# zsc/ARTalk

Hardware: AMD Instinct MI355X
Metric: motion frames/sec (25 fps clips) at batch=32 per GPU (higher is better)
Workload: dtype f32 (operands split into 2 fp16, 3 fp16 MFMA products per fp32 product, fp32 accumulate)

## Files before the change

artalk_amd/capi.py:

```python
from __future__ import annotations

import ctypes as C
import os

from .config import ARTalkConfig

_HERE = os.path.dirname(os.path.abspath(__file__))
LIB_PATH = os.environ.get("ARTALK_LIB") or os.path.join(_HERE, "libartalk_hip.so")

OK, EINVAL, EKEY, EMISSING, EHIP, ESTATE, ECAPACITY, EBUSY = 0, -1, -2, -3, -4, -5, -6, -7
DTYPE_F32, DTYPE_I64 = 0, 1

SYMBOLS = [
    "artalk_create", "artalk_destroy", "artalk_last_error", "artalk_set_tensor", "artalk_finalize_weights",
    "artalk_reserve", "artalk_workspace_bytes", "artalk_weight_bytes", "artalk_infer", "artalk_get_status", "artalk_poll_status", "artalk_last_ticket", "artalk_get_status_of", "artalk_style_encode", "artalk_stream_begin", "artalk_stream_chunk", "artalk_stream_end", "artalk_savgol", "artalk_flame_create", "artalk_flame_verts", "artalk_flame_destroy", "artalk_flame_last_error",
    "artalk_set_profiling", "artalk_get_profile", "artalk_get_kernel_sums", "artalk_set_graphs", "artalk_graph_count", "artalk_set_cu_mask", "artalk_set_audit", "artalk_get_audit", "artalk_calibrate", "artalk_reset_scales", "artalk_get_scales", "artalk_scale_sites", "artalk_get_site_scales", "artalk_set_site_scales", "artalk_set_tap", "artalk_tap_layout", "artalk_set_precision",
    "artalk_op_gemm", "artalk_op_gemm_ex", "artalk_op_gemm_bf16", "artalk_op_gemm_f16s", "artalk_op_pack_split", "artalk_op_gemm_f16s_packed", "artalk_op_release_scratch", "artalk_op_gemm_p8_plan", "artalk_op_create_masked_stream", "artalk_op_destroy_stream", "artalk_op_mfma_f32_peak", "artalk_op_layernorm", "artalk_op_attention", "artalk_op_w2v_front", "artalk_op_resample_mean", "artalk_op_pool_silu",
    "artalk_op_bsq_history",
    "artalk_sessions_reserve", "artalk_session_open", "artalk_session_step", "artalk_session_close", "artalk_session_count",
    "artalk_session_smooth", "artalk_op_savgol_stream", "artalk_op_session_smooth_check",
    "artalk_op_pack_split_ex", "artalk_op_layernorm_ex", "artalk_op_gemm_f16s_packed_ex", "artalk_op_gemm_f16s_ex", "artalk_op_attention_ex", "artalk_op_w2v_front_ex", "artalk_op_pool_silu_ex", "artalk_op_posconv_p8_ex",
    "artalk_op_bsq_history_ex", "artalk_op_ar_bits_next", "artalk_op_vq_embed", "artalk_op_ar_begin", "artalk_op_dec_input", "artalk_op_dec_finish", "artalk_op_enc_input_zero", "artalk_op_style_input", "artalk_op_add_row", "artalk_op_style_finish", "artalk_op_broadcast16", "artalk_op_session_gather", "artalk_op_session_scatter", "artalk_op_absmax",
    "artalk_op_gemm_rows", "artalk_op_layernorm_rows", "artalk_op_attention_rows", "artalk_op_gemm_rows_layout", "artalk_op_rows_dry_run",
    "artalk_op_w2v_front_rows", "artalk_op_pool_silu_rows", "artalk_op_posconv_rows",
]


class ArtalkConfigStruct(C.Structure):
    _fields_ = [
        ("ar_depth", C.c_int32), ("ar_heads", C.c_int32),
        ("vae_depth", C.c_int32), ("vae_heads", C.c_int32), ("vae_hidden", C.c_int32),
        ("code_dim", C.c_int32), ("motion_dim", C.c_int32),
        ("n_levels", C.c_int32), ("patch_nums", C.c_int32 * 8),
        ("w2v_layers", C.c_int32), ("w2v_hidden", C.c_int32), ("w2v_heads", C.c_int32), ("w2v_ffn", C.c_int32),
        ("w2v_n_conv", C.c_int32), ("w2v_conv_kernel", C.c_int32 * 8), ("w2v_conv_stride", C.c_int32 * 8),
        ("w2v_conv_dim", C.c_int32),
        ("w2v_pos_kernel", C.c_int32), ("w2v_pos_groups", C.c_int32),
        ("w2v_ln_eps", C.c_float),
        ("style_dim", C.c_int32), ("style_heads", C.c_int32), ("style_layers", C.c_int32), ("style_ffn", C.c_int32),
# ... 79 lines not shown
    L.artalk_destroy.restype = None
    L.artalk_last_error.argtypes = [vp]
    L.artalk_last_error.restype = C.c_char_p
    L.artalk_set_tensor.argtypes = [vp, C.c_char_p, vp, i32, i32, C.POINTER(i64)]
    L.artalk_set_tensor.restype = i32
    L.artalk_finalize_weights.argtypes = [vp]
    L.artalk_finalize_weights.restype = i32
    L.artalk_reserve.argtypes = [vp, i32, i32]
    L.artalk_reserve.restype = i32
    L.artalk_workspace_bytes.argtypes = [vp]
    L.artalk_workspace_bytes.restype = i64
    L.artalk_weight_bytes.argtypes = [vp]
    L.artalk_weight_bytes.restype = i64
    L.artalk_infer.argtypes = [vp, vp, i64, C.POINTER(i64), i32, vp, vp, vp, i64, vp, vp, vp, vp]
    L.artalk_infer.restype = i32
    L.artalk_get_status.argtypes = [vp, C.POINTER(C.c_int), vp]
    L.artalk_get_status.restype = i32
    L.artalk_poll_status.argtypes = [vp, C.POINTER(C.c_int)]
    L.artalk_poll_status.restype = i32
    L.artalk_last_ticket.argtypes = [vp]
    L.artalk_last_ticket.restype = C.c_longlong
    L.artalk_get_status_of.argtypes = [vp, C.c_longlong, C.POINTER(C.c_int)]
    L.artalk_get_status_of.restype = i32
    L.artalk_style_encode.argtypes = [vp, vp, i32, vp, vp]
    L.artalk_style_encode.restype = i32
    L.artalk_stream_begin.argtypes = [vp, i32, vp, vp, vp]
    L.artalk_stream_begin.restype = i32
    L.artalk_stream_end.argtypes = [vp]
    L.artalk_stream_end.restype = i32
    L.artalk_stream_chunk.argtypes = [vp, vp, i64, vp, i64, vp]
# ... 173 lines not shown
```

artalk_amd/csrc/engine.hip:

```cpp
#include "kernels.h"
#include "../../include/artalk_hip.h"

#include <hip/hip_ext.h>
#include <rocprofiler-sdk-roctx/roctx.h>

#include <algorithm>
#include <cmath>
#include <cstdio>
#include <cstdlib>
#include <cstring>
#include <map>
#include <set>
#include <string>
#include <vector>

using namespace artalk;

namespace artalk {
thread_local KernelTimer* g_ktimer = nullptr;
bool ktimer_events(hipEvent_t* e0, hipEvent_t* e1) {
    KernelTimer* t = g_ktimer;
    if (!t) return false;
    while (t->pool.size() < t->used + 2) {
        hipEvent_t e = nullptr;
// ... 116 lines not shown
        std::vector<float*> blocks;
        std::vector<int64_t> owner;
        struct Open { int slot = 0; int64_t seen = 0; bool smooth_done = false; };
        std::map<int64_t, Open> open;
        std::set<int64_t> ended_by_scales;
        int64_t next_id = 1;
        void* smooth_tab = nullptr; int64_t smooth_cap = 0;
    } sess;
    int64_t sess_carry_off() const { return slot_carry_off(cfg.code_dim); }
    int64_t sess_slot_floats() const { return sess_carry_off() + (kSavgolCarry * (int64_t)cfg.motion_dim + 3) / 4 * 4; }
    float* sess_slot(int i) const { return sess.blocks[i / kSessBlock] + (int64_t)(i % kSessBlock) * sess_slot_floats(); }
    Workspace* view = nullptr;
    bool sticky_error = false;
    int n_conv = 0; int conv_T[8]{}; int conv_S[8]{};
    int Tw = 0, Ts = 0;
    int ada_n = 0;
    int pn[kMaxLv]{}, off[kMaxLv + 1]{};
    float *conv0_w = nullptr, *conv_b[8]{}, *conv_lnw[8]{}, *conv_lnb[8]{}, *conv_w[8]{};
    float *fp_lnw = nullptr, *fp_lnb = nullptr, *fp_w = nullptr, *fp_b = nullptr;
    float *pos_w = nullptr, *pos_b = nullptr, *enc_lnw = nullptr, *enc_lnb = nullptr;
    std::vector<W2VLayer> w2v;
    float *ada_w = nullptr, *ada_b = nullptr;
    float *ar_qkv_w = nullptr, *ar_qkv_b = nullptr;
    std::vector<ARLayer> ar;
    float *logits_w = nullptr, *logits_b = nullptr, *vq_w = nullptr, *vq_b = nullptr, *sc_w = nullptr, *sc_b = nullptr;
    float *null_style = nullptr, *lvl_pos = nullptr, *prev_lvl_pos = nullptr;
    float *enc_pos = nullptr, *dec_pos = nullptr, *vae_mean = nullptr, *vae_std = nullptr;
    VAESide enc, dec;
    float *st_mean = nullptr, *st_std = nullptr, *st_pe = nullptr, *st_proj_w = nullptr, *st_proj_b = nullptr;
    std::vector<StyleLayer> style;
// ... 274 lines not shown
    auto st = m->site_of.find(ex);
    if (st == m->site_of.end()) { m->err = "internal: audited exponent is not in the site table"; m->sticky_error = true; return; }
    const std::string& name = m->sites[st->second].name;
    auto it = m->audit_index.find(name);
    int idx;
    if (it == m->audit_index.end()) {
        if ((int)m->audit_names.size() >= kAuditSlots) return;
        idx = (int)m->audit_names.size();
        m->audit_names.push_back(name);
        m->audit_exp.push_back(ex);
        m->audit_index.emplace(name, idx);
    } else idx = it->second;
    launch_absmax(buf, rows, cols & ~7, ld, is_p8 ? 1 : 0, m->audit_vals + idx, s, junk_period, junk_from, ex ? *ex : kActExp);
}

bool gemm(artalk_model* m, const GemmArgs& g0, hipStream_t s, const LnArgs* fuse_ln = nullptr) {
    GemmArgs g = g0;
    g.graph_tag = m->in_body ? 1 : 0;
    g.cus = m->n_cus;
    g.status = m->precision == 1 ? (m->view ? m->view->status : m->ws.status) : nullptr;
    if (m->precision == 1 && !g.exact) g.Wp = packed_of(m, g.W);
    if (m->precision == 2 && !g.exact) {
        g.Wb = bf16_of(m, g.W);
        if (!g.Wb || ((unsigned long long)g.Wb & 15) || (g.ldw & 7)) {
            m->err = "internal: bf16 GEMM without an aligned bf16 weight copy"; m->sticky_error = true; return false;
        }
        if (g.a_packed) { m->err = "internal: P8 activation handed to a bf16 GEMM"; m->sticky_error = true; return false; }
    }
    const Workspace& cw = m->view ? *m->view : m->ws;
    const GemmPolicy pol{m->precision, false, cw.splitk, cw.splitk_floats, m->splitk_tiles, m->splitk_target};
    const GemmPlan plan = plan_gemm(g, pol, fuse_ln);
    if (g.a_packed && plan.path == GEMM_F32) { m->err = "internal: P8 activation handed to an fp32 GEMM"; m->sticky_error = true; return false; }
    const bool timed = m->profiling && plan.dominant && !m->in_body;
    size_t i0 = 0, i1 = 0;
    if (timed) next_event(m, s, &i0);
    run_gemm(g, plan, fuse_ln, s);
    if (timed) {
        next_event(m, s, &i1);
        m->dom_events.emplace_back(i0, gemm_flops(g));
    }
    return plan.fused_ln;
}

enum { TAP_BLK0_IN = 0, TAP_BLK0_OUT = kNTok * kE, TAP_BLKL_OUT = 2 * kNTok * kE, TAP_PREV_IN = 3 * kNTok * kE,
       TAP_LOGITS = 4 * kNTok * kE, TAP_DEC_OUT = 4 * kNTok * kE + kNTok * 64, TAP_SLOT = 4 * kNTok * kE + kNTok * 64 + 200 * 106 };
void tap_copy(artalk_model* m, int field, int row0, const float* src, int rows, int cols, int B, hipStream_t s) {
    if (!m->tap || m->in_graph_body || m->tap_chunk >= m->tap_maxch || B > m->tap_B) return;
    float* dst = m->tap + ((long)m->tap_chunk * m->tap_B) * TAP_SLOT + field + (long)row0 * cols;
    (void)hipMemcpy2DAsync(dst, (size_t)TAP_SLOT * 4, src, (size_t)rows * cols * 4, (size_t)rows * cols * 4, B, hipMemcpyDeviceToDevice, s);
}

enum { LF_EXACT = 1, LF_A_P8 = 2, LF_C_P8 = 4 };
void linear(artalk_model* m, const float* A, long lda, const float* W, const float* bias, float* C, long ldc, int M, int N, int K,
            int act, const float* R, hipStream_t s, int flags = 0, float* c2 = nullptr, int a_exp = kActExp, int c_exp = kActExp) {
    GemmArgs g;
    g.c2 = c2; g.a_exp = a_exp; g.c_exp = c_exp;
    g.exact = flags & LF_EXACT; g.a_packed = (flags & LF_A_P8) ? 1 : 0; g.c_p8 = (flags & LF_C_P8) ? 1 : 0;
    g.A = A; g.lda = lda; g.W = W; g.ldw = K; g.bias = bias; g.C = C; g.ldc = ldc; g.M = M; g.N = N; g.K = K; g.act = act;
    g.R = R; g.ldr = ldc;
    gemm(m, g, s);
}

void layernorm(const float* X, float* Y, const float* w, const float* b, int M, int D, float eps, int act, hipStream_t s, int out_p8 = 0,
               int* status = nullptr, int junk_period = 0, int junk_from = 0, int p8_exp = kActExp) {
    LnArgs a;
    a.out_p8 = out_p8; a.p8_exp = p8_exp; a.status = out_p8 ? status : nullptr; a.junk_period = junk_period; a.junk_from = junk_from;
    a.X = X; a.ldx = D; a.Y = Y; a.ldy = D; a.w = w; a.b = b; a.M = M; a.D = D; a.eps = eps; a.act = act;
    launch_layernorm(a, s);
}

void run_wav2vec(artalk_model* m, const float* audio, int c0, int n, float* out_w2v, hipStream_t s) {
    const artalk_config& c = m->cfg;
    Workspace& w = m->ws;
    const int CD = c.w2v_conv_dim, Hs = c.w2v_hidden;
    const int p8 = m->precision == 1 ? 1 : 0;
    const int AP = p8 ? LF_A_P8 : 0;
    Range r_w2v("artalk.wav2vec2");
    roctxRangePushA("artalk.wav2vec2.conv_stack");
    kbucket(m, KB_CONV);
    launch_audio_normalize(audio, w.src_off + c0, w.xnorm, n, kSamplesPerChunk, s);
    SiteExps& ex = m->ex;
    launch_conv0(w.xnorm, kSamplesPerChunk, m->conv0_w, m->conv_b[0], m->conv_lnw[0], m->conv_lnb[0], w.convA, n, m->conv_T[0],
                 m->conv_S[0], s, p8, w.status, ex.conv[0]);
    audit(m, w.convA, n * m->conv_S[0], CD, CD, p8, s, &ex.conv[0], m->conv_S[0], m->conv_T[0]);
    float* src = w.convA; float* dst = w.convB;
    for (int i = 1; i < c.w2v_n_conv; ++i) {
        const int M = n * m->conv_S[i];
        linear(m, src, (long)c.w2v_conv_stride[i] * CD, m->conv_w[i], m->conv_b[i], dst, CD, M, CD, c.w2v_conv_kernel[i] * CD,
               ACT_NONE, nullptr, s, AP, nullptr, ex.conv[i - 1]);
        layernorm(dst, dst, m->conv_lnw[i], m->conv_lnb[i], M, CD, 1e-5f, ACT_GELU_ERF, s, (p8 && i + 1 < c.w2v_n_conv) ? 1 : 0, w.status,
                  m->conv_S[i], m->conv_T[i], ex.conv[i]);
        if (i + 1 < c.w2v_n_conv) audit(m, dst, M, CD, CD, p8, s, &ex.conv[i], m->conv_S[i], m->conv_T[i]);
        std::swap(src, dst);
    }
    stage_mark(m, s, PB_CONV);
    roctxRangePop();
    Range r_enc("artalk.wav2vec2.encoder");
    kbucket(m, KB_ENC);
    const int M = n * m->Ts;
    const int JP = m->Ts, JF = m->Tw;
    layernorm(src, dst, m->fp_lnw, m->fp_lnb, M, CD, c.w2v_ln_eps, ACT_NONE, s, p8, w.status, JP, JF, ex.fp_ln);
    audit(m, dst, M, CD, CD, p8, s, &ex.fp_ln, JP, JF);
    linear(m, dst, CD, m->fp_w, m->fp_b, w.h0, Hs, M, Hs, CD, ACT_NONE, nullptr, s, AP, nullptr, ex.fp_ln);
    audit(m, w.h0, M, Hs, Hs, false, s, &ex.posconv_in, JP, JF);
    {
        const int cg = Hs / c.w2v_pos_groups;
        GemmArgs g;
        g.A = w.h0; g.lda = Hs; g.W = m->pos_w; g.ldw = (long)cg * c.w2v_pos_kernel; g.bias = m->pos_b; g.C = w.h1; g.ldc = Hs; g.R = w.h0; g.ldr = Hs;
        g.M = M; g.act = ACT_GELU_ERF; g.a_exp = ex.posconv_in;
// ... 537 lines not shown
        if (m->stream_B > 0) { m->stream_B = 0; m->stream_scales_ended = true; }
        end_sessions_by_scales(m);
        m->ex = next;
    }
    m->scales_changed = 0;
    for (size_t i = 0; i < sizeof(SiteExps) / sizeof(int); ++i) m->scales_changed += a[i] != kActExp;
    return changed;
}

int call_stream(artalk_model* m, void* stream, hipStream_t* s) {
    (void)hipSetDevice(m->device);
    if (!stream && !m->own_stream) HIPCHK(m, hipStreamCreate(&m->own_stream));
    *s = stream ? (hipStream_t)stream : m->own_stream;
    return ARTALK_OK;
}
int check_has_style(artalk_model* m, const float* style_motion_dev, const uint8_t* has_style, int B, bool* encode) {
    *encode = false;
    for (int b = 0; style_motion_dev && has_style && b < B; ++b) {
        if (has_style[b] > 2) return fail(m, ARTALK_EINVAL, "has_style entries must be 0, 1 or 2");
        *encode |= has_style[b] == 1;
    }
    return ARTALK_OK;
}
int begin_clips(artalk_model* m, hipStream_t s, int B, const float* style_motion_dev, const uint8_t* has_style, bool encode_style,
                artalk_model::Stage* stg) {
    Workspace& w = m->ws;
    if (!has_style) style_motion_dev = nullptr;
    if (style_motion_dev) {
        std::memcpy(stg->has, has_style, (size_t)B);
        HIPCHK(m, hipMemcpyAsync(w.has_style, stg->has, B, hipMemcpyHostToDevice, s));
// ... 458 lines not shown
    int n = 0;
    for (uint32_t w : m->cu_mask) n += __builtin_popcount(w);
    if (n_words > 0 && n < 8) { m->cu_mask.clear(); m->n_cus = 0; return fail(m, ARTALK_EINVAL, "a CU partition needs at least 8 compute units"); }
    int dev_cus = 0;
    if (hipDeviceGetAttribute(&dev_cus, hipDeviceAttributeMultiprocessorCount, m->device) == hipSuccess && dev_cus > 0) n = std::min(n, dev_cus);
    m->n_cus = n;
    for (int i = 0; i < 3; ++i) {
        if (m->side_stream[i]) { (void)hipStreamDestroy(m->side_stream[i]); m->side_stream[i] = nullptr; }
        if (m->join_ev[i]) { (void)hipEventDestroy(m->join_ev[i]); m->join_ev[i] = nullptr; }
    }
    drop_graphs(m);
    m->invalidate_init_hist();
    return ARTALK_OK;
}

int artalk_infer(artalk_model* m, const float* audio_dev, int64_t audio_clip_stride, const int64_t* n_chunks, int B,
                 const float* style_motion_dev, const uint8_t* has_style, float* out_motion_dev, int64_t out_clip_stride,
                 uint8_t* out_bits_dev, uint8_t* out_hist_bits_dev, float* out_w2v_dev, void* stream) {
    if (!m || !audio_dev || !n_chunks || !out_motion_dev || B <= 0) return ARTALK_EINVAL;
    if (!m->finalized) return fail(m, ARTALK_ESTATE, "artalk_infer before artalk_finalize_weights");
    hipStream_t s;
    if (int rc = call_stream(m, stream, &s)) return rc;
    const artalk_config& c = m->cfg;
    int64_t C = 0, maxch = n_chunks[0];
    for (int b = 0; b < B; ++b) {
        if (n_chunks[b] <= 0 || (b > 0 && n_chunks[b] > n_chunks[b - 1])) return fail(m, ARTALK_EINVAL, "n_chunks must be positive and non-increasing");
        C += n_chunks[b];
    }
    bool encode_style;
    if (int rc = check_has_style(m, style_motion_dev, has_style, B, &encode_style)) return rc;
    if (m->tap && (B > m->tap_B || maxch > m->tap_maxch)) return fail(m, ARTALK_EINVAL, "the tap buffer (artalk_set_tap) is smaller than this call");
    if (B > m->ws.maxB || C > m->ws.maxC) { if (int rc = reserve(m, B, (int)C)) return rc; }
    Workspace& w = m->ws;
    artalk_model::Stage* stg = nullptr;
    if (int rc = next_stage(m, &stg)) return rc;
    long* src = stg->src;
    std::vector<int> base((size_t)maxch + 1, 0), Bj((size_t)maxch, 0);
    {
        int idx = 0;
        for (int64_t j = 0; j < maxch; ++j) {
            base[j] = idx;
            for (int b = 0; b < B && n_chunks[b] > j; ++b) { src[idx++] = (long)b * audio_clip_stride + (long)j * kSamplesPerChunk; Bj[j]++; }
        }
        base[maxch] = idx;
    }
    HIPCHK(m, hipMemcpyAsync(w.src_off, src, C * sizeof(long), hipMemcpyHostToDevice, s));
    m->stream_B = 0; m->stream_scales_ended = false;
    m->ev_used = 0; m->dom_events.clear(); m->marks.clear(); m->prof_stream = s;
    struct TimerScope { bool on; TimerScope(artalk_model* x) : on(x->profiling == 3) { if (on) { x->ktimer.used = 0; x->ktimer.recs.clear(); x->ktimer.bucket = KB_OTHER; g_ktimer = &x->ktimer; } }
                        ~TimerScope() { if (on) g_ktimer = nullptr; } } timer_scope(m);
    if (int rc = begin_clips(m, s, B, style_motion_dev, has_style, encode_style, stg)) return rc;
    for (int c0 = 0; c0 < C; c0 += w.G) run_wav2vec(m, audio_dev, c0, (int)std::min<int64_t>(w.G, C - c0), out_w2v_dev, s);
    if (int rc = run_init_history(m, B, s)) return rc;
    const size_t bits_row = (size_t)kNTok * c.code_dim;
    if (out_hist_bits_dev)
        HIPCHK(m, hipMemcpy2DAsync(out_hist_bits_dev, (size_t)(maxch + 1) * bits_row, w.hist_bits, bits_row, bits_row, B,
                                   hipMemcpyDeviceToDevice, s));
    stage_mark(m, s, PB_VAE);
    for (int64_t j = 0; j < maxch; ++j) {
// ... 42 lines not shown
    if (int rc = ensure_stage(m, m->ws.maxB, m->ws.maxC)) return rc;
    artalk_model::Stage* stg = nullptr;
    if (int rc = next_stage(m, &stg)) return rc;
    {
        ProfilingOff quiet(m);
        if (int rc = begin_clips(m, s, B, style_motion_dev, has_style, encode_style, stg)) return rc;
        if (int rc = run_init_history(m, B, s)) return rc;
    }
    m->stream_B = B; m->stream_scales_ended = false;
    if (int rc = publish_status(m, s)) return rc;
    return ARTALK_OK;
}

int artalk_stream_chunk(artalk_model* m, const float* audio_dev, int64_t chunk_stride, float* out_motion_dev, int64_t out_stride,
                        void* stream) {
    if (!m || !audio_dev || !out_motion_dev) return ARTALK_EINVAL;
    if (m->stream_B <= 0)
        return fail(m, ARTALK_ESTATE, m->stream_scales_ended ? "the site scales changed since artalk_stream_begin; begin again"
                                                             : "artalk_stream_chunk before artalk_stream_begin");
    hipStream_t s;
    if (int rc = call_stream(m, stream, &s)) return rc;
    const int B = m->stream_B;
    Workspace& w = m->ws;
    if (B > w.maxB) return fail(m, ARTALK_ESTATE, "workspace was re-reserved since artalk_stream_begin; begin again");
    artalk_model::Stage* stg = nullptr;
    if (int rc = next_stage(m, &stg)) return rc;
    for (int b = 0; b < B; ++b) stg->src[b] = (long)b * chunk_stride;
    HIPCHK(m, hipMemcpyAsync(w.src_off, stg->src, B * sizeof(long), hipMemcpyHostToDevice, s));
    HIPCHK(m, hipEventRecord(stg->done, s));
    stg->used = true;
    ProfilingOff quiet(m);
    for (int c0 = 0; c0 < B; c0 += w.G) run_wav2vec(m, audio_dev, c0, std::min(w.G, B - c0), nullptr, s);
    if (int rc = chunk_step(m, s, 0, B, B, m->tap_maxch, out_motion_dev, out_stride)) return rc;
    if (int rc = publish_status(m, s)) return rc;
    return ARTALK_OK;
}

int artalk_stream_end(artalk_model* m) {
    if (!m) return ARTALK_EINVAL;
// ... 32 lines not shown
        if (int rc = begin_clips(m, s, n, style_motion_dev, has_style, encode_style, stg)) return rc;
        if (int rc = run_init_history(m, n, s)) return rc;
    }
    launch_session_scatter(m->ws.sess_slots, session_rows(m), n, true, s);
    if (int rc = publish_status(m, s)) return rc;
    for (int i = 0; i < n; ++i) {
        ids_out[i] = ss.next_id++;
        ss.owner[slot[i]] = ids_out[i];
        ss.open.emplace(ids_out[i], artalk_model::Sessions::Open{slot[i]});
    }
    return ARTALK_OK;
}

int artalk_session_step(artalk_model* m, const int64_t* ids, int n, const float* audio_dev, int64_t chunk_stride, float* out_motion_dev,
                        int64_t out_stride, uint8_t* out_bits_dev, uint8_t* out_hist_bits_dev, void* stream) {
    if (!m || !ids || n <= 0 || !audio_dev || !out_motion_dev) return ARTALK_EINVAL;
    artalk_model::Sessions& ss = m->sess;
    std::vector<int> slot((size_t)n);
    std::set<int64_t> seen;
    for (int i = 0; i < n; ++i) {
        const auto it = ss.open.find(ids[i]);
        if (it == ss.open.end()) {
            if (ss.ended_by_scales.count(ids[i]))
                return fail(m, ARTALK_ESTATE, "session " + std::to_string(ids[i]) + ": the site scales changed since artalk_session_open; open the session again");
            return fail(m, ARTALK_EINVAL, "artalk_session_step: " + std::to_string(ids[i]) + " is not an open session");
        }
        if (!seen.insert(ids[i]).second) return fail(m, ARTALK_EINVAL, "artalk_session_step: session " + std::to_string(ids[i]) + " is listed twice");
        slot[i] = it->second.slot;
    }
    hipStream_t s;
    if (int rc = call_stream(m, stream, &s)) return rc;
// ... 921 lines not shown
```

artalk_amd/csrc/kernels.h:

```cpp
#pragma once
#include <hip/hip_runtime.h>
#include <climits>
#include <cstdint>

#include <hip/hip_ext.h>
#include <utility>
#include <vector>

namespace artalk {

struct KernelTimer {
    int bucket = 0;
    std::vector<hipEvent_t> pool; size_t used = 0;
    std::vector<std::pair<int, size_t>> recs;
};
extern thread_local KernelTimer* g_ktimer;
bool ktimer_events(hipEvent_t* e0, hipEvent_t* e1);
#define ARTALK_LAUNCH(kernel, grid, block, lds, stream, ...)                                                          \
    do {                                                                                                              \
        hipEvent_t kt_e0_ = nullptr, kt_e1_ = nullptr;                                                                \
        if (artalk::g_ktimer && artalk::ktimer_events(&kt_e0_, &kt_e1_))                                              \
            hipExtLaunchKernelGGL(kernel, grid, block, lds, stream, kt_e0_, kt_e1_, 0, __VA_ARGS__);                  \
        else                                                                                                          \
            hipLaunchKernelGGL(kernel, grid, block, lds, stream, __VA_ARGS__);                                        \
// ... 98 lines not shown
    int l2norm = 0; const float* qscale = nullptr;
    int split_q = 0, split_k = 0;
    int out_p8 = 0;
    int split16 = 0;
    int qkv_p8 = 0;
    int qkv_exp = 4, o_exp = 4;
    int* status = nullptr;
    int cus = 0;
};
void launch_attention(const AttnArgs& a, hipStream_t s);
void attention_prepare();

void launch_audio_normalize(const float* audio, const long* src_off, float* xnorm, int n_chunks, int n, hipStream_t s);
void launch_conv0(const float* xnorm, int n, const float* w , const float* bias, const float* lnw,
                  const float* lnb, float* Y, int n_chunks, int T, int row_stride, hipStream_t s, int out_p8 = 0, int* status = nullptr, int p8_exp = kActExp);
void launch_pool_silu(const float* X, int x_tstride, int T, float* Y, int n_chunks, const int* patch_nums, int n_lvls,
                      int D, hipStream_t s, int out_p8 = 0, int* status = nullptr, int p8_exp = kActExp);

void launch_ar_bits_next(const float* logits, uint8_t* bits, float* fhat, float* nextfeat, int B, int level, hipStream_t s,
                         int* status = nullptr);
void launch_vq_embed(const float* feat, int n, const float* We, const float* be, const float* pos, float* X, int xrows,
                     int xoff, const float* style_cond, const float* pos0, int B, hipStream_t s);
void launch_ar_begin(const float* style_cond, const float* lvlpos, float* x0, float* fhat, int B, hipStream_t s);
void launch_dec_input(const float* prev_fdec, const float* fhat, const uint8_t* bits, const float* dpos, float* X,
                      int B, hipStream_t s);
void launch_dec_finish(const float* dec , const float* mean, const float* stdv, const float* epos,
                       float* out, long out_bstride, int chunk, float* E, int B, hipStream_t s, int* status = nullptr);
void launch_enc_input_zero(const float* mean, const float* stdv, const float* epos, float* E, int B, hipStream_t s);
void launch_broadcast16(const void* src, void* dst, long bytes, int B, hipStream_t s);
struct SessionRows {
// ... 30 lines not shown
```

artalk_amd/csrc/w2v_front.hip:

```cpp
#include "common.h"

namespace artalk {

__global__ __launch_bounds__(1024) void audio_normalize_kernel(const float* __restrict__ audio, const long* __restrict__ src_off,
                                                               float* __restrict__ xn, int n) {
    __shared__ double red[16];
    __shared__ float stat[2];
    const int c = blockIdx.x, tid = threadIdx.x, lane = tid & 63, wv = tid >> 6;
    const float* x = audio + src_off[c];
    double s = 0.0;
    for (int i = tid; i < n; i += 1024) s += (double)x[i];
#pragma unroll
    for (int o = 32; o > 0; o >>= 1) s += __shfl_xor(s, o, 64);
    if (lane == 0) red[wv] = s;
    __syncthreads();
    if (tid == 0) {
        double t = 0.0;
        for (int i = 0; i < 16; ++i) t += red[i];
        stat[0] = (float)(t / n);
    }
    __syncthreads();
    const double mean = (double)stat[0];
    double q = 0.0;
    for (int i = tid; i < n; i += 1024) { const double d = (double)x[i] - mean; q += d * d; }
// ... 68 lines not shown
            store_p8x4_pair(y, 256 + lane * 4, o[2].x, o[2].y, o[3].x, o[3].y, status, p8_exp);
        } else {
            f32x4 lo = {o[0].x, o[0].y, o[1].x, o[1].y}, hi = {o[2].x, o[2].y, o[3].x, o[3].y};
            *reinterpret_cast<f32x4*>(y + lane * 4) = lo;
            *reinterpret_cast<f32x4*>(y + 256 + lane * 4) = hi;
        }
    }
}

void launch_conv0(const float* xnorm, int n, const float* w, const float* bias, const float* lnw, const float* lnb,
                  float* Y, int n_chunks, int T, int row_stride, hipStream_t s, int out_p8, int* status, int p8_exp) {
    if (n_chunks <= 0) return;
    ARTALK_LAUNCH(conv0_kernel, dim3(128, n_chunks), dim3(256), 0, s, xnorm, n, w, bias, lnw, lnb, Y, T, row_stride, status, out_p8, p8_exp);
}

struct PoolLevels { int n; int pn[8]; };

__global__ __launch_bounds__(256) void pool_silu_kernel(const float* __restrict__ X, int x_tstride, int T, float* __restrict__ Y,
                                                        PoolLevels lv, int ntok, int D, int out_p8, int* __restrict__ status, int p8_exp) {
    const int tok = blockIdx.x, c = blockIdx.y;
    int p = 0, i = tok;
    while (i >= lv.pn[p]) { i -= lv.pn[p]; ++p; }
    const int pn = lv.pn[p];
    const int t0 = (i * T) / pn, t1 = ((i + 1) * T + pn - 1) / pn;
    const float inv = (float)(t1 - t0);
    for (int d = threadIdx.x * 4; d < D; d += 256 * 4) {
        f32x4 s = {0.f, 0.f, 0.f, 0.f};
        for (int t = t0; t < t1; ++t) s += *reinterpret_cast<const f32x4*>(X + ((long)c * x_tstride + t) * D + d);
        f32x4 o;
#pragma unroll
// ... 48 lines not shown
```

artalk_amd/model.py:

```python
from __future__ import annotations

import ctypes as C
import math
from typing import List, Optional, Sequence

import numpy as np
import torch

from . import capi
from .config import ARTalkConfig

SCALES_FORMAT = "artalk-site-scales/1"
SCALE_EXP_MIN, SCALE_EXP_MAX = -8, 4


def check_scales(sites, names: Sequence[str]) -> List[int]:
    if not isinstance(sites, dict):
        raise ValueError("site scales must be a {site name: exponent} dict")
    missing = [n for n in names if n not in sites]
    extra = [n for n in sites if n not in set(names)]
    if missing or extra:
        raise ValueError("the site scales do not match this model's site table ({} missing, e.g. {}; {} extra, e.g. {}): they belong to "
                         "another architecture".format(len(missing), missing[:3], len(extra), extra[:3]))
    exps = []
# ... 301 lines not shown

    def set_precision(self, mode):
        names = {0: "f32", 1: "f16x3", 2: "bf16"}
        code = {"f32": 0, "f16x3": 1, "bf16": 2}.get(mode, mode)
        if code not in names:
            raise ValueError(f"precision mode must be 'f32', 'f16x3' or 'bf16' (got {mode!r})")
        code = int(code)
        self._precision = names[code]
        self._latched_f32 = False
        if self._h is not None and self._loaded:
            rc = capi.lib().artalk_set_precision(self._h, int(code))
            if rc == capi.EINVAL:
                raise ValueError("precision mode must be 'f32', 'f16x3' or 'bf16'")
            if rc != capi.OK:
                raise RuntimeError(f"artalk_set_precision({code}) failed ({rc}): {self._err()}")

    def set_graphs(self, on: bool, branches: int = 0, splitk_tiles: int = 0, splitk_target: int = 0):
        capi.lib().artalk_set_graphs(self._h, int(bool(on)) | (int(branches) << 8) | ((splitk_tiles // 16) << 16) | ((splitk_target // 16) << 24))

    def graph_count(self):
        n = C.c_longlong(0)
        held = capi.lib().artalk_graph_count(self._h, C.byref(n))
        return int(held), int(n.value)

    def set_cu_mask(self, words: Optional[Sequence[int]]):
        if not self._loaded:
            raise RuntimeError("load_state_dict must be called before set_cu_mask")
        L = capi.lib()
        self.stream_end()
        with torch.cuda.device(self._device):
# ... 111 lines not shown
        self._stream_style = style_motions
        self._stream_fed = [0] * self._n_streams

    @torch.no_grad()
    def stream_chunk(self, audio_chunks: torch.Tensor, n_valid: Optional[Sequence[int]] = None):
        B = getattr(self, "_n_streams", 0)
        if B <= 0:
            raise RuntimeError("stream_chunk before stream_begin")
        assert audio_chunks.shape == (B, self.cfg.samples_per_chunk), f"expected ({B}, {self.cfg.samples_per_chunk}) samples"
        dev = self._device
        with torch.cuda.device(dev):
            x = audio_chunks.to(device=dev, dtype=torch.float32).contiguous()
            out = torch.empty(B, 100, self.cfg.motion_dim, dtype=torch.float32, device=dev)
            caller = torch.cuda.current_stream()
            self._stream.wait_stream(caller)
            rc = capi.lib().artalk_stream_chunk(self._h, capi.ptr(x), x.stride(0), capi.ptr(out), out.stride(0),
                                                C.c_void_p(self._stream.cuda_stream))
            caller.wait_stream(self._stream)
            x.record_stream(self._stream)
            out.record_stream(self._stream)
        if rc != capi.OK:
            raise RuntimeError("artalk_stream_chunk failed: " + self._err())
        if self._precision == "f16x3" and self.check_finite and self.status() != 0:
            self.stream_end()
            if self.auto_calibrate:
                try:
                    changed = self.calibrate([x[b] for b in range(B)], self._stream_style)
                except RuntimeError:
                    changed = 0
                if changed > 0:
# ... 88 lines not shown
        assert len({sess.id for sess in sessions}) == n, "a session is listed twice"
        assert tuple(audio_chunks.shape) == (n, self.cfg.samples_per_chunk), f"expected ({n}, {self.cfg.samples_per_chunk}) samples"
        dev = self._device
        ids = (C.c_int64 * n)(*[sess.id for sess in sessions])
        with torch.cuda.device(dev):
            x = audio_chunks.to(device=dev, dtype=torch.float32).contiguous()
            out = torch.empty(n, 100, self.cfg.motion_dim, dtype=torch.float32, device=dev)
            bits = hist = None
            if return_aux:
                bits = torch.empty(n, 181, self.cfg.code_dim, dtype=torch.uint8, device=dev)
                hist = torch.empty(n, 181, self.cfg.code_dim, dtype=torch.uint8, device=dev)
            if self._stream is None:
                self._stream = torch.cuda.Stream(device=dev)
            caller = torch.cuda.current_stream()
            self._stream.wait_stream(caller)
            rc = capi.lib().artalk_session_step(self._h, ids, n, capi.ptr(x), x.stride(0), capi.ptr(out), out.stride(0),
                                                capi.ptr(bits), capi.ptr(hist), C.c_void_p(self._stream.cuda_stream))
            caller.wait_stream(self._stream)
            for t in (x, out, bits, hist):
                if t is not None:
                    t.record_stream(self._stream)
        if rc != capi.OK:
            msg = self._err()
            self._sync_sessions()
            raise RuntimeError("artalk_session_step failed: " + msg)
        self._n_streams = 0
        if self._precision == "f16x3" and self.check_finite and self.status() != 0:
            styles = [sess.style_motion for sess in sessions]
            changed = 0
            if self.auto_calibrate:
# ... 148 lines not shown
                out = torch.zeros(B, maxch * 100, self.cfg.motion_dim, dtype=torch.float32, device=dev)
                bits = hist = w2v = None
                if return_aux:
                    bits = torch.zeros(B, maxch, 181, 32, dtype=torch.uint8, device=dev)
                    hist = torch.zeros(B, maxch + 1, 181, 32, dtype=torch.uint8, device=dev)
                    w2v = torch.zeros(total, 199, self.cfg.cond_dim, dtype=torch.float32, device=dev)
            tap_t = None
            if taps and return_aux:
                lay = (C.c_int64 * 7)()
                L.artalk_tap_layout(lay, 7)
                with torch.cuda.stream(self._stream):
                    tap_t = torch.zeros(maxch * B, int(lay[6]), dtype=torch.float32, device=dev)
                if L.artalk_set_tap(self._h, capi.ptr(tap_t), B, maxch) != capi.OK:
                    raise RuntimeError("artalk_set_tap failed: " + self._err())
            nch_sorted = (C.c_int64 * B)(*[nch[i] for i in order])
            rc = L.artalk_infer(self._h, capi.ptr(audio_pad), audio_pad.stride(0), nch_sorted, B, capi.ptr(style_t),
                                C.cast(has, C.c_void_p) if has is not None else None, capi.ptr(out), out.stride(0),
                                capi.ptr(bits), capi.ptr(hist), capi.ptr(w2v), C.c_void_p(self._stream.cuda_stream))
            caller.wait_stream(self._stream)
            if tap_t is not None:
                L.artalk_set_tap(self._h, None, 0, 0)
            for t in (audio_pad, style_t):
                if t is not None:
                    t.record_stream(self._stream)
            for t in (out, bits, hist, w2v, tap_t):
                if t is not None:
                    t.record_stream(caller)
            if rc != capi.OK:
                raise RuntimeError("artalk_infer failed ({}): {}".format(rc, self._err()))
            if check and self._precision == "f16x3" and self.check_finite and self.status() != 0:
# ... 39 lines not shown
```

include/artalk_hip.h:

```cpp
#ifndef ARTALK_HIP_H
#define ARTALK_HIP_H

#include <stdint.h>

#ifdef __cplusplus
extern "C" {
#endif

#define ARTALK_OK 0
#define ARTALK_EINVAL (-1)
#define ARTALK_EKEY (-2)
#define ARTALK_EMISSING (-3)
#define ARTALK_EHIP (-4)
#define ARTALK_ESTATE (-5)
#define ARTALK_ECAPACITY (-6)
#define ARTALK_EBUSY (-7)

#define ARTALK_DTYPE_F32 0
#define ARTALK_DTYPE_I64 1

typedef struct artalk_model artalk_model;

typedef struct artalk_config {
    int32_t ar_depth, ar_heads;
// ... 9 lines not shown

int artalk_create(int device_id, const artalk_config* cfg, artalk_model** out);
void artalk_destroy(artalk_model* m);
const char* artalk_last_error(const artalk_model* m);

int artalk_set_tensor(artalk_model* m, const char* key, const void* host_ptr, int dtype, int ndim, const int64_t* shape);
int artalk_finalize_weights(artalk_model* m);

int artalk_reserve(artalk_model* m, int max_batch, int max_total_chunks);
int64_t artalk_workspace_bytes(const artalk_model* m);
int64_t artalk_weight_bytes(const artalk_model* m);

int artalk_infer(artalk_model* m, const float* audio_dev, int64_t audio_clip_stride, const int64_t* n_chunks, int B,
                 const float* style_motion_dev, const uint8_t* has_style, float* out_motion_dev, int64_t out_clip_stride,
                 uint8_t* out_bits_dev, uint8_t* out_hist_bits_dev, float* out_w2v_dev, void* stream);

int artalk_style_encode(artalk_model* m, const float* style_motion_dev, int n, float* out_cond_dev, void* stream);

int artalk_stream_end(artalk_model* m);
int artalk_stream_begin(artalk_model* m, int B, const float* style_motion_dev, const uint8_t* has_style, void* stream);
int artalk_stream_chunk(artalk_model* m, const float* audio_dev, int64_t chunk_stride, float* out_motion_dev, int64_t out_stride,
                        void* stream);

int artalk_sessions_reserve(artalk_model* m, int max_sessions);
int artalk_session_open(artalk_model* m, int n, const float* style_motion_dev, const uint8_t* has_style, int64_t* ids_out, void* stream);
int artalk_session_step(artalk_model* m, const int64_t* ids, int n, const float* audio_dev, int64_t chunk_stride, float* out_motion_dev,
                        int64_t out_stride, uint8_t* out_bits_dev, uint8_t* out_hist_bits_dev, void* stream);
int artalk_session_close(artalk_model* m, const int64_t* ids, int n);
int artalk_session_count(const artalk_model* m);
int artalk_session_smooth(artalk_model* m, const int64_t* ids, int n, const float* raw_dev, int64_t raw_stride, const int* n_frames,
// ... 147 lines not shown
```

Measured before the change: 105,400.

## Skip wav2vec conv front work on zero-padded tail samples of final chunks

Passes per-clip valid sample counts into the engine and groups chunks into up to four runs by bucketed valid length. For runs whose audio ends early it computes a reduced conv geometry, runs conv0 and the strided conv GEMMs over only the rows that depend on real samples, then expands the last valid row into the padded positions. This is meant to remove conv-stack compute on padding in partial chunks, at the cost of more kernel launches per run and extra planning checks. Outputs in the padded region are replicated rather than computed, so exactness depends on the padding region not affecting downstream results.

```diff
diff --git a/artalk_amd/capi.py b/artalk_amd/capi.py
--- a/artalk_amd/capi.py
+++ b/artalk_amd/capi.py
@@ -23,6 +23,7 @@
     "artalk_op_bsq_history_ex", "artalk_op_ar_bits_next", "artalk_op_vq_embed", "artalk_op_ar_begin", "artalk_op_dec_input", "artalk_op_dec_finish", "artalk_op_enc_input_zero", "artalk_op_style_input", "artalk_op_add_row", "artalk_op_style_finish", "artalk_op_broadcast16", "artalk_op_session_gather", "artalk_op_session_scatter", "artalk_op_absmax",
     "artalk_op_gemm_rows", "artalk_op_layernorm_rows", "artalk_op_attention_rows", "artalk_op_gemm_rows_layout", "artalk_op_rows_dry_run",
     "artalk_op_w2v_front_rows", "artalk_op_pool_silu_rows", "artalk_op_posconv_rows",
+    "artalk_set_valid_samples", "artalk_set_skip_padding", "artalk_skip_padding_runs", "artalk_conv_tail_geometry", "artalk_conv_run_classes",
 ]
 
 
@@ -132,6 +133,17 @@
     L.artalk_weight_bytes.restype = i64
     L.artalk_infer.argtypes = [vp, vp, i64, C.POINTER(i64), i32, vp, vp, vp, i64, vp, vp, vp, vp]
     L.artalk_infer.restype = i32
+    if hasattr(L, "artalk_set_valid_samples"):
+        L.artalk_set_valid_samples.argtypes = [vp, C.POINTER(i64), i32]
+        L.artalk_set_valid_samples.restype = i32
+        L.artalk_set_skip_padding.argtypes = [vp, i32]
+        L.artalk_set_skip_padding.restype = i32
+        L.artalk_skip_padding_runs.argtypes = [vp]
+        L.artalk_skip_padding_runs.restype = i64
+        L.artalk_conv_tail_geometry.argtypes = [C.POINTER(ArtalkConfigStruct), i32, C.POINTER(i32), C.POINTER(i32), i32]
+        L.artalk_conv_tail_geometry.restype = i32
+        L.artalk_conv_run_classes.argtypes = [C.POINTER(i32), i32, C.POINTER(i32), C.POINTER(i32), C.POINTER(i32), i32]
+        L.artalk_conv_run_classes.restype = i32
     L.artalk_get_status.argtypes = [vp, C.POINTER(C.c_int), vp]
     L.artalk_get_status.restype = i32
     L.artalk_poll_status.argtypes = [vp, C.POINTER(C.c_int)]
diff --git a/artalk_amd/csrc/engine.hip b/artalk_amd/csrc/engine.hip
--- a/artalk_amd/csrc/engine.hip
+++ b/artalk_amd/csrc/engine.hip
@@ -154,6 +154,10 @@
     bool sticky_error = false;
     int n_conv = 0; int conv_T[8]{}; int conv_S[8]{};
     int Tw = 0, Ts = 0;
+    bool skip_padding = true;
+    std::vector<int64_t> next_valid;
+    std::vector<int> chunk_valid;
+    int64_t short_runs = 0;
     int ada_n = 0;
     int pn[kMaxLv]{}, off[kMaxLv + 1]{};
     float *conv0_w = nullptr, *conv_b[8]{}, *conv_lnw[8]{}, *conv_lnb[8]{}, *conv_w[8]{};
@@ -458,8 +462,7 @@
     launch_absmax(buf, rows, cols & ~7, ld, is_p8 ? 1 : 0, m->audit_vals + idx, s, junk_period, junk_from, ex ? *ex : kActExp);
 }
 
-bool gemm(artalk_model* m, const GemmArgs& g0, hipStream_t s, const LnArgs* fuse_ln = nullptr) {
-    GemmArgs g = g0;
+bool plan_model_gemm(artalk_model* m, GemmArgs& g, GemmPlan* plan_out, const LnArgs* fuse_ln) {
     g.graph_tag = m->in_body ? 1 : 0;
     g.cus = m->n_cus;
     g.status = m->precision == 1 ? (m->view ? m->view->status : m->ws.status) : nullptr;
@@ -473,8 +476,15 @@
     }
     const Workspace& cw = m->view ? *m->view : m->ws;
     const GemmPolicy pol{m->precision, false, cw.splitk, cw.splitk_floats, m->splitk_tiles, m->splitk_target};
-    const GemmPlan plan = plan_gemm(g, pol, fuse_ln);
-    if (g.a_packed && plan.path == GEMM_F32) { m->err = "internal: P8 activation handed to an fp32 GEMM"; m->sticky_error = true; return false; }
+    *plan_out = plan_gemm(g, pol, fuse_ln);
+    if (g.a_packed && plan_out->path == GEMM_F32) { m->err = "internal: P8 activation handed to an fp32 GEMM"; m->sticky_error = true; return false; }
+    return true;
+}
+
+bool gemm(artalk_model* m, const GemmArgs& g0, hipStream_t s, const LnArgs* fuse_ln = nullptr) {
+    GemmArgs g = g0;
+    GemmPlan plan;
+    if (!plan_model_gemm(m, g, &plan, fuse_ln)) return false;
     const bool timed = m->profiling && plan.dominant && !m->in_body;
     size_t i0 = 0, i1 = 0;
     if (timed) next_event(m, s, &i0);
@@ -495,14 +505,18 @@
 }
 
 enum { LF_EXACT = 1, LF_A_P8 = 2, LF_C_P8 = 4 };
-void linear(artalk_model* m, const float* A, long lda, const float* W, const float* bias, float* C, long ldc, int M, int N, int K,
-            int act, const float* R, hipStream_t s, int flags = 0, float* c2 = nullptr, int a_exp = kActExp, int c_exp = kActExp) {
+GemmArgs linear_args(const float* A, long lda, const float* W, const float* bias, float* C, long ldc, int M, int N, int K, int act,
+                     const float* R, int flags = 0, float* c2 = nullptr, int a_exp = kActExp, int c_exp = kActExp) {
     GemmArgs g;
     g.c2 = c2; g.a_exp = a_exp; g.c_exp = c_exp;
     g.exact = flags & LF_EXACT; g.a_packed = (flags & LF_A_P8) ? 1 : 0; g.c_p8 = (flags & LF_C_P8) ? 1 : 0;
     g.A = A; g.lda = lda; g.W = W; g.ldw = K; g.bias = bias; g.C = C; g.ldc = ldc; g.M = M; g.N = N; g.K = K; g.act = act;
     g.R = R; g.ldr = ldc;
-    gemm(m, g, s);
+    return g;
+}
+void linear(artalk_model* m, const float* A, long lda, const float* W, const float* bias, float* C, long ldc, int M, int N, int K,
+            int act, const float* R, hipStream_t s, int flags = 0, float* c2 = nullptr, int a_exp = kActExp, int c_exp = kActExp) {
+    gemm(m, linear_args(A, lda, W, bias, C, ldc, M, N, K, act, R, flags, c2, a_exp, c_exp), s);
 }
 
 void layernorm(const float* X, float* Y, const float* w, const float* b, int M, int D, float eps, int act, hipStream_t s, int out_p8 = 0,
@@ -511,6 +525,90 @@
     a.out_p8 = out_p8; a.p8_exp = p8_exp; a.status = out_p8 ? status : nullptr; a.junk_period = junk_period; a.junk_from = junk_from;
     a.X = X; a.ldx = D; a.Y = Y; a.ldy = D; a.w = w; a.b = b; a.M = M; a.D = D; a.eps = eps; a.act = act;
     launch_layernorm(a, s);
+}
+
+bool conv_tail_geometry(const artalk_config& c, int v, int* T, int* S) {
+    const int L = c.w2v_n_conv;
+    if (L < 2 || L > 8 || v < 1 || v > kSamplesPerChunk) return false;
+    int full[8], cst[8], t = kSamplesPerChunk;
+    for (int i = 0; i < L; ++i) {
+        const int k = c.w2v_conv_kernel[i], st = c.w2v_conv_stride[i];
+        if (k < 1 || st < 1 || (i > 0 && st != 2) || t < k) return false;
+        t = (t - k) / st + 1;
+        full[i] = t;
+        cst[i] = i == 0 ? (v + st - 1) / st : (cst[i - 1] + 1) / 2;
+    }
+    T[L - 1] = std::min(full[L - 1], cst[L - 1] + 1);
+    for (int i = L - 1; i > 0; --i) T[i - 1] = std::min(full[i - 1], std::max(cst[i - 1] + 1, 2 * (T[i] - 1) + c.w2v_conv_kernel[i]));
+    int s = T[L - 1] + 1;
+    for (int i = 0; i < L; ++i) s = std::max(s, (T[i] + (1 << (L - 1 - i)) - 1) >> (L - 1 - i));
+    for (int i = L - 1; i >= 0; --i) { S[i] = s; s *= 2; }
+    return true;
+}
+
+struct ConvRun { int r0 = 0, n = 0, v = 0; bool tail = false; int T[8]{}, S[8]{}; };
+constexpr int kTailBucket = 3200;
+constexpr int kMaxConvRuns = 4;
+
+bool conv_gemms_order_kept(artalk_model* m, int rn, const int* S, int n) {
+    const artalk_config& c = m->cfg;
+    const int CD = c.w2v_conv_dim, AP = m->precision == 1 ? LF_A_P8 : 0;
+    for (int i = 1; i < c.w2v_n_conv; ++i) {
+        GemmPlan plan[2];
+        for (int f = 0; f < 2; ++f) {
+            GemmArgs g = linear_args(i & 1 ? m->ws.convA : m->ws.convB, (long)c.w2v_conv_stride[i] * CD, m->conv_w[i], m->conv_b[i],
+                                     i & 1 ? m->ws.convB : m->ws.convA, CD, f ? n * m->conv_S[i] : rn * S[i], CD, c.w2v_conv_kernel[i] * CD,
+                                     ACT_NONE, nullptr, AP, nullptr, m->ex.conv[i - 1]);
+            if (!plan_model_gemm(m, g, &plan[f], nullptr) || g.splitk != 1) return false;
+        }
+        if (plan[0].path != GEMM_P8 || plan[1].path != GEMM_P8) return false;
+    }
+    return true;
+}
+
+void merge_conv_runs(std::vector<ConvRun>& runs, size_t i) {
+    runs[i].n += runs[i + 1].n; runs[i].v = std::max(runs[i].v, runs[i + 1].v);
+    runs.erase(runs.begin() + i + 1);
+}
+std::vector<ConvRun> conv_run_classes(const int* valid, int n) {
+    std::vector<ConvRun> runs;
+    for (int k = 0; k < n; ++k) {
+        const int v = std::min(kSamplesPerChunk, (std::max(valid[k], 1) + kTailBucket - 1) / kTailBucket * kTailBucket);
+        if (!runs.empty() && runs.back().v == v) { ++runs.back().n; continue; }
+        ConvRun r; r.r0 = k; r.n = 1; r.v = v;
+        runs.push_back(r);
+    }
+    while ((int)runs.size() > kMaxConvRuns) {
+        size_t best = 0; int64_t cost = INT64_MAX;
+        for (size_t i = 0; i + 1 < runs.size(); ++i) {
+            const int v = std::max(runs[i].v, runs[i + 1].v);
+            const int64_t ci = (int64_t)runs[i].n * (v - runs[i].v) + (int64_t)runs[i + 1].n * (v - runs[i + 1].v);
+            if (ci < cost) { cost = ci; best = i; }
+        }
+        merge_conv_runs(runs, best);
+    }
+    return runs;
+}
+
+std::vector<ConvRun> conv_runs(artalk_model* m, int c0, int n) {
+    const int L = m->cfg.w2v_n_conv;
+    const bool skip = m->skip_padding && (int)m->chunk_valid.size() >= c0 + n &&
+                      m->conv_S[(L - 1) % 2] >= 2 * m->Ts;
+    std::vector<ConvRun> runs;
+    if (skip) runs = conv_run_classes(m->chunk_valid.data() + c0, n);
+    else { runs.assign(1, ConvRun()); runs[0].n = n; runs[0].v = kSamplesPerChunk; }
+    for (ConvRun& r : runs) {
+        r.tail = r.v < kSamplesPerChunk && conv_tail_geometry(m->cfg, r.v, r.T, r.S) && r.T[L - 1] < m->conv_T[L - 1] &&
+                 conv_gemms_order_kept(m, r.n, r.S, n);
+        if (!r.tail) r.v = kSamplesPerChunk;
+    }
+    for (size_t i = 0; i + 1 < runs.size();)
+        if (!runs[i].tail && !runs[i + 1].tail) merge_conv_runs(runs, i); else ++i;
+    bool kept = true;
+    for (const ConvRun& r : runs)
+        if (!r.tail && r.n < n) kept = kept && conv_gemms_order_kept(m, r.n, m->conv_S, n);
+    if (!kept) { runs.assign(1, ConvRun()); runs[0].n = n; runs[0].v = kSamplesPerChunk; }
+    return runs;
 }
 
 void run_wav2vec(artalk_model* m, const float* audio, int c0, int n, float* out_w2v, hipStream_t s) {
@@ -524,19 +622,33 @@
     kbucket(m, KB_CONV);
     launch_audio_normalize(audio, w.src_off + c0, w.xnorm, n, kSamplesPerChunk, s);
     SiteExps& ex = m->ex;
-    launch_conv0(w.xnorm, kSamplesPerChunk, m->conv0_w, m->conv_b[0], m->conv_lnw[0], m->conv_lnb[0], w.convA, n, m->conv_T[0],
-                 m->conv_S[0], s, p8, w.status, ex.conv[0]);
-    audit(m, w.convA, n * m->conv_S[0], CD, CD, p8, s, &ex.conv[0], m->conv_S[0], m->conv_T[0]);
-    float* src = w.convA; float* dst = w.convB;
-    for (int i = 1; i < c.w2v_n_conv; ++i) {
-        const int M = n * m->conv_S[i];
-        linear(m, src, (long)c.w2v_conv_stride[i] * CD, m->conv_w[i], m->conv_b[i], dst, CD, M, CD, c.w2v_conv_kernel[i] * CD,
-               ACT_NONE, nullptr, s, AP, nullptr, ex.conv[i - 1]);
-        layernorm(dst, dst, m->conv_lnw[i], m->conv_lnb[i], M, CD, 1e-5f, ACT_GELU_ERF, s, (p8 && i + 1 < c.w2v_n_conv) ? 1 : 0, w.status,
-                  m->conv_S[i], m->conv_T[i], ex.conv[i]);
-        if (i + 1 < c.w2v_n_conv) audit(m, dst, M, CD, CD, p8, s, &ex.conv[i], m->conv_S[i], m->conv_T[i]);
-        std::swap(src, dst);
-    }
+    const int L = c.w2v_n_conv;
+    float* const last = (L - 1) % 2 ? w.convB : w.convA;
+    for (const ConvRun& run : conv_runs(m, c0, n)) {
+        const int* T = run.tail ? run.T : m->conv_T;
+        const int* S = run.tail ? run.S : m->conv_S;
+        const int r0 = run.r0, rn = run.n;
+        float* src = w.convA + (long)r0 * m->conv_S[0] * CD;
+        launch_conv0(w.xnorm + (long)r0 * kSamplesPerChunk, kSamplesPerChunk, m->conv0_w, m->conv_b[0], m->conv_lnw[0], m->conv_lnb[0], src,
+                     rn, T[0], S[0], s, p8, w.status, ex.conv[0]);
+        audit(m, src, rn * S[0], CD, CD, p8, s, &ex.conv[0], S[0], T[0]);
+        for (int i = 1; i < L; ++i) {
+            const int M = rn * S[i];
+            float* dst = (i & 1 ? w.convB : w.convA) + (run.tail && i == L - 1 ? (long)w.G * m->Ts : (long)r0 * m->conv_S[i]) * CD;
+            linear(m, src, (long)c.w2v_conv_stride[i] * CD, m->conv_w[i], m->conv_b[i], dst, CD, M, CD, c.w2v_conv_kernel[i] * CD,
+                   ACT_NONE, nullptr, s, AP, nullptr, ex.conv[i - 1]);
+            layernorm(dst, dst, m->conv_lnw[i], m->conv_lnb[i], M, CD, 1e-5f, ACT_GELU_ERF, s, (p8 && i + 1 < L) ? 1 : 0, w.status,
+                      S[i], T[i], ex.conv[i]);
+            if (i + 1 < L) audit(m, dst, M, CD, CD, p8, s, &ex.conv[i], S[i], T[i]);
+            src = dst;
+        }
+        if (run.tail) {
+            launch_conv_tail_expand(src, S[L - 1], T[L - 1], last + (long)r0 * m->Ts * CD, m->Ts, m->Tw, rn, CD, s);
+            ++m->short_runs;
+        }
+    }
+    float* src = last;
+    float* dst = last == w.convA ? w.convB : w.convA;
     stage_mark(m, s, PB_CONV);
     roctxRangePop();
     Range r_enc("artalk.wav2vec2.encoder");
@@ -1104,6 +1216,17 @@
     *s = stream ? (hipStream_t)stream : m->own_stream;
     return ARTALK_OK;
 }
+std::vector<int64_t> take_valid_samples(artalk_model* m) {
+    std::vector<int64_t> v;
+    v.swap(m->next_valid);
+    return v;
+}
+int set_chunk_valid(artalk_model* m, const std::vector<int64_t>& valid, int n) {
+    if (!valid.empty() && (int64_t)valid.size() != n) return fail(m, ARTALK_EINVAL, "artalk_set_valid_samples: the count differs from this call's streams");
+    m->chunk_valid.clear();
+    for (int64_t v : valid) m->chunk_valid.push_back((int)std::min<int64_t>(std::max<int64_t>(v, 0), kSamplesPerChunk));
+    return ARTALK_OK;
+}
 int check_has_style(artalk_model* m, const float* style_motion_dev, const uint8_t* has_style, int B, bool* encode) {
     *encode = false;
     for (int b = 0; style_motion_dev && has_style && b < B; ++b) {
@@ -1592,10 +1715,35 @@
     return ARTALK_OK;
 }
 
+int artalk_conv_tail_geometry(const artalk_config* cfg, int valid_samples, int* T_out, int* S_out, int n) {
+    if (!cfg || !T_out || !S_out || n < cfg->w2v_n_conv) return ARTALK_EINVAL;
+    return conv_tail_geometry(*cfg, valid_samples, T_out, S_out) ? ARTALK_OK : ARTALK_EINVAL;
+}
+int artalk_conv_run_classes(const int32_t* valid_samples, int n, int* r0_out, int* n_out, int* v_out, int max_runs) {
+    if (!valid_samples || n <= 0 || !r0_out || !n_out || !v_out || max_runs < kMaxConvRuns) return ARTALK_EINVAL;
+    const std::vector<ConvRun> runs = conv_run_classes(valid_samples, n);
+    for (size_t i = 0; i < runs.size(); ++i) { r0_out[i] = runs[i].r0; n_out[i] = runs[i].n; v_out[i] = runs[i].v; }
+    return (int)runs.size();
+}
+int artalk_set_skip_padding(artalk_model* m, int on) {
+    if (!m) return ARTALK_EINVAL;
+    m->skip_padding = on != 0;
+    return ARTALK_OK;
+}
+int artalk_set_valid_samples(artalk_model* m, const int64_t* n_samples, int n) {
+    if (!m || n < 0 || (n > 0 && !n_samples)) return ARTALK_EINVAL;
+    m->next_valid.assign(n_samples, n_samples + n);
+    return ARTALK_OK;
+}
+int64_t artalk_skip_padding_runs(const artalk_model* m) { return m ? m->short_runs : ARTALK_EINVAL; }
+
 int artalk_infer(artalk_model* m, const float* audio_dev, int64_t audio_clip_stride, const int64_t* n_chunks, int B,
                  const float* style_motion_dev, const uint8_t* has_style, float* out_motion_dev, int64_t out_clip_stride,
                  uint8_t* out_bits_dev, uint8_t* out_hist_bits_dev, float* out_w2v_dev, void* stream) {
-    if (!m || !audio_dev || !n_chunks || !out_motion_dev || B <= 0) return ARTALK_EINVAL;
+    if (!m) return ARTALK_EINVAL;
+    const std::vector<int64_t> valid = take_valid_samples(m);
+    if (!audio_dev || !n_chunks || !out_motion_dev || B <= 0) return ARTALK_EINVAL;
+    if (!valid.empty() && (int64_t)valid.size() != B) return fail(m, ARTALK_EINVAL, "artalk_set_valid_samples: the count differs from this call's clips");
     if (!m->finalized) return fail(m, ARTALK_ESTATE, "artalk_infer before artalk_finalize_weights");
     hipStream_t s;
     if (int rc = call_stream(m, stream, &s)) return rc;
@@ -1621,6 +1769,10 @@
             for (int b = 0; b < B && n_chunks[b] > j; ++b) { src[idx++] = (long)b * audio_clip_stride + (long)j * kSamplesPerChunk; Bj[j]++; }
         }
         base[maxch] = idx;
+        m->chunk_valid.clear();
+        for (int64_t j = 0; !valid.empty() && j < maxch; ++j)
+            for (int b = 0; b < B && n_chunks[b] > j; ++b)
+                m->chunk_valid.push_back((int)std::min<int64_t>(std::max<int64_t>(valid[b] - j * kSamplesPerChunk, 0), kSamplesPerChunk));
     }
     HIPCHK(m, hipMemcpyAsync(w.src_off, src, C * sizeof(long), hipMemcpyHostToDevice, s));
     m->stream_B = 0; m->stream_scales_ended = false;
@@ -1693,7 +1845,9 @@
 
 int artalk_stream_chunk(artalk_model* m, const float* audio_dev, int64_t chunk_stride, float* out_motion_dev, int64_t out_stride,
                         void* stream) {
-    if (!m || !audio_dev || !out_motion_dev) return ARTALK_EINVAL;
+    if (!m) return ARTALK_EINVAL;
+    const std::vector<int64_t> valid = take_valid_samples(m);
+    if (!audio_dev || !out_motion_dev) return ARTALK_EINVAL;
     if (m->stream_B <= 0)
         return fail(m, ARTALK_ESTATE, m->stream_scales_ended ? "the site scales changed since artalk_stream_begin; begin again"
                                                              : "artalk_stream_chunk before artalk_stream_begin");
@@ -1702,6 +1856,7 @@
     const int B = m->stream_B;
     Workspace& w = m->ws;
     if (B > w.maxB) return fail(m, ARTALK_ESTATE, "workspace was re-reserved since artalk_stream_begin; begin again");
+    if (int rc = set_chunk_valid(m, valid, B)) return rc;
     artalk_model::Stage* stg = nullptr;
     if (int rc = next_stage(m, &stg)) return rc;
     for (int b = 0; b < B; ++b) stg->src[b] = (long)b * chunk_stride;
@@ -1764,7 +1919,10 @@
 
 int artalk_session_step(artalk_model* m, const int64_t* ids, int n, const float* audio_dev, int64_t chunk_stride, float* out_motion_dev,
                         int64_t out_stride, uint8_t* out_bits_dev, uint8_t* out_hist_bits_dev, void* stream) {
-    if (!m || !ids || n <= 0 || !audio_dev || !out_motion_dev) return ARTALK_EINVAL;
+    if (!m) return ARTALK_EINVAL;
+    const std::vector<int64_t> valid = take_valid_samples(m);
+    if (!ids || n <= 0 || !audio_dev || !out_motion_dev) return ARTALK_EINVAL;
+    if (int rc = set_chunk_valid(m, valid, n)) return rc;
     artalk_model::Sessions& ss = m->sess;
     std::vector<int> slot((size_t)n);
     std::set<int64_t> seen;
diff --git a/artalk_amd/csrc/kernels.h b/artalk_amd/csrc/kernels.h
--- a/artalk_amd/csrc/kernels.h
+++ b/artalk_amd/csrc/kernels.h
@@ -136,6 +136,7 @@
 void launch_audio_normalize(const float* audio, const long* src_off, float* xnorm, int n_chunks, int n, hipStream_t s);
 void launch_conv0(const float* xnorm, int n, const float* w , const float* bias, const float* lnw,
                   const float* lnb, float* Y, int n_chunks, int T, int row_stride, hipStream_t s, int out_p8 = 0, int* status = nullptr, int p8_exp = kActExp);
+void launch_conv_tail_expand(const float* X, int x_stride, int n_rows, float* Y, int y_stride, int T, int n_chunks, int D, hipStream_t s);
 void launch_pool_silu(const float* X, int x_tstride, int T, float* Y, int n_chunks, const int* patch_nums, int n_lvls,
                       int D, hipStream_t s, int out_p8 = 0, int* status = nullptr, int p8_exp = kActExp);
 
diff --git a/artalk_amd/csrc/w2v_front.hip b/artalk_amd/csrc/w2v_front.hip
--- a/artalk_amd/csrc/w2v_front.hip
+++ b/artalk_amd/csrc/w2v_front.hip
@@ -106,6 +106,20 @@
     ARTALK_LAUNCH(conv0_kernel, dim3(128, n_chunks), dim3(256), 0, s, xnorm, n, w, bias, lnw, lnb, Y, T, row_stride, status, out_p8, p8_exp);
 }
 
+__global__ __launch_bounds__(128) void conv_tail_expand_kernel(const float* __restrict__ X, int x_stride, int n_rows, float* __restrict__ Y,
+                                                               int y_stride, int T, int D) {
+    const int t = blockIdx.x, c = blockIdx.y;
+    const f32x4* x = reinterpret_cast<const f32x4*>(X + ((long)c * x_stride + min(t, n_rows - 1)) * D);
+    f32x4* y = reinterpret_cast<f32x4*>(Y + ((long)c * y_stride + t) * D);
+    const f32x4 zero = {0.f, 0.f, 0.f, 0.f};
+    for (int i = threadIdx.x; i < D / 4; i += 128) y[i] = t < T ? x[i] : zero;
+}
+
+void launch_conv_tail_expand(const float* X, int x_stride, int n_rows, float* Y, int y_stride, int T, int n_chunks, int D, hipStream_t s) {
+    if (n_chunks <= 0 || n_rows < 1 || n_rows > T || T > y_stride || (D & 3)) return;
+    ARTALK_LAUNCH(conv_tail_expand_kernel, dim3(y_stride, n_chunks), dim3(128), 0, s, X, x_stride, n_rows, Y, y_stride, T, D);
+}
+
 struct PoolLevels { int n; int pn[8]; };
 
 __global__ __launch_bounds__(256) void pool_silu_kernel(const float* __restrict__ X, int x_tstride, int T, float* __restrict__ Y,
diff --git a/artalk_amd/model.py b/artalk_amd/model.py
--- a/artalk_amd/model.py
+++ b/artalk_amd/model.py
@@ -339,6 +339,30 @@
                 raise ValueError("precision mode must be 'f32', 'f16x3' or 'bf16'")
             if rc != capi.OK:
                 raise RuntimeError(f"artalk_set_precision({code}) failed ({rc}): {self._err()}")
+
+    def set_skip_padding(self, on: bool):
+        L = capi.lib()
+        if not hasattr(L, "artalk_set_skip_padding"):
+            raise RuntimeError("this build of the library has no artalk_set_skip_padding")
+        if L.artalk_set_skip_padding(self._h, int(bool(on))) != capi.OK:
+            raise RuntimeError("artalk_set_skip_padding failed: " + self._err())
+
+    def skip_padding_runs(self) -> int:
+        L = capi.lib()
+        if not hasattr(L, "artalk_skip_padding_runs"):
+            return 0
+        n = int(L.artalk_skip_padding_runs(self._h))
+        if n < 0:
+            raise RuntimeError("artalk_skip_padding_runs failed")
+        return n
+
+    def _pass_valid_samples(self, counts: Optional[Sequence[int]]):
+        L = capi.lib()
+        if counts is None or not hasattr(L, "artalk_set_valid_samples"):
+            return
+        arr = (C.c_int64 * len(counts))(*[int(v) for v in counts])
+        if L.artalk_set_valid_samples(self._h, arr, len(counts)) != capi.OK:
+            raise RuntimeError("artalk_set_valid_samples failed: " + self._err())
 
     def set_graphs(self, on: bool, branches: int = 0, splitk_tiles: int = 0, splitk_target: int = 0):
         capi.lib().artalk_set_graphs(self._h, int(bool(on)) | (int(branches) << 8) | ((splitk_tiles // 16) << 16) | ((splitk_target // 16) << 24))
@@ -480,6 +504,7 @@
             out = torch.empty(B, 100, self.cfg.motion_dim, dtype=torch.float32, device=dev)
             caller = torch.cuda.current_stream()
             self._stream.wait_stream(caller)
+            self._pass_valid_samples(n_valid)
             rc = capi.lib().artalk_stream_chunk(self._h, capi.ptr(x), x.stride(0), capi.ptr(out), out.stride(0),
                                                 C.c_void_p(self._stream.cuda_stream))
             caller.wait_stream(self._stream)
@@ -598,6 +623,7 @@
                 self._stream = torch.cuda.Stream(device=dev)
             caller = torch.cuda.current_stream()
             self._stream.wait_stream(caller)
+            self._pass_valid_samples(n_valid)
             rc = capi.lib().artalk_session_step(self._h, ids, n, capi.ptr(x), x.stride(0), capi.ptr(out), out.stride(0),
                                                 capi.ptr(bits), capi.ptr(hist), C.c_void_p(self._stream.cuda_stream))
             caller.wait_stream(self._stream)
@@ -776,6 +802,7 @@
                 if L.artalk_set_tap(self._h, capi.ptr(tap_t), B, maxch) != capi.OK:
                     raise RuntimeError("artalk_set_tap failed: " + self._err())
             nch_sorted = (C.c_int64 * B)(*[nch[i] for i in order])
+            self._pass_valid_samples([n_samples[i] for i in order])
             rc = L.artalk_infer(self._h, capi.ptr(audio_pad), audio_pad.stride(0), nch_sorted, B, capi.ptr(style_t),
                                 C.cast(has, C.c_void_p) if has is not None else None, capi.ptr(out), out.stride(0),
                                 capi.ptr(bits), capi.ptr(hist), capi.ptr(w2v), C.c_void_p(self._stream.cuda_stream))
diff --git a/include/artalk_hip.h b/include/artalk_hip.h
--- a/include/artalk_hip.h
+++ b/include/artalk_hip.h
@@ -47,6 +47,12 @@
 int artalk_infer(artalk_model* m, const float* audio_dev, int64_t audio_clip_stride, const int64_t* n_chunks, int B,
                  const float* style_motion_dev, const uint8_t* has_style, float* out_motion_dev, int64_t out_clip_stride,
                  uint8_t* out_bits_dev, uint8_t* out_hist_bits_dev, float* out_w2v_dev, void* stream);
+
+int artalk_set_valid_samples(artalk_model* m, const int64_t* n_samples, int n);
+int artalk_set_skip_padding(artalk_model* m, int on);
+int64_t artalk_skip_padding_runs(const artalk_model* m);
+int artalk_conv_tail_geometry(const artalk_config* cfg, int valid_samples, int* T_out, int* S_out, int n);
+int artalk_conv_run_classes(const int32_t* valid_samples, int n, int* r0_out, int* n_out, int* v_out, int max_runs);
 
 int artalk_style_encode(artalk_model* m, const float* style_motion_dev, int n, float* out_cond_dev, void* stream);
 
```

Result: no change. 106,400, median of 6 (+1.0%).
